# Blaizzy/mlx-audio

Hardware: NVIDIA H100
Metric: audio-sec/sec Kokoro-82M TTS (128-phoneme utterance, 9.75 s) (higher is better)
Workload: dtype bf16x2

## Files before the change

### mlx_audio_b200/csrc/lstm.cu

```cuda
#include "common.cuh"
#include <cooperative_groups.h>
#include <stdlib.h>
namespace cg = cooperative_groups;

namespace {

constexpr int LH = 256, NCTA = 8, UPC = LH / NCTA;

__global__ void __cluster_dims__(NCTA, 1, 1) __launch_bounds__(256, 1)
lstm_bidir_kernel(const float* __restrict__ xproj, const float* __restrict__ wh, float* __restrict__ out,
                  int64_t out_ld, int T) {
  cg::cluster_group cluster = cg::this_cluster();
  const int rank = (int)cluster.block_rank();
  const int dir = blockIdx.y, b = blockIdx.z;
  const int tid = threadIdx.x, half = tid & 1, r = tid >> 1;
  const int gate = r >> 5, unit = r & 31;
  const int grow = gate * LH + rank * UPC + unit;
  __shared__ __align__(16) float hbuf[2][LH];
  __shared__ float gates[4 * UPC];

  float w[128];
  {
    const float* wp = wh + ((int64_t)dir * 4 * LH + grow) * LH + half * 128;
#pragma unroll
    for (int j = 0; j < 128; j += 4) {
      float4 t = *reinterpret_cast<const float4*>(wp + j);
      w[j] = t.x; w[j + 1] = t.y; w[j + 2] = t.z; w[j + 3] = t.w;
    }
  }
  for (int i = tid; i < 2 * LH; i += 256) (&hbuf[0][0])[i] = 0.f;
  float c = 0.f;
  const float* xp_base = xproj + (int64_t)b * T * 2 * 4 * LH + (int64_t)dir * 4 * LH + grow;
  float xp_cur = 0.f;
  if (half == 0 && T > 0) xp_cur = __ldg(xp_base + (int64_t)(dir == 0 ? 0 : T - 1) * 2 * 4 * LH);
  cluster.sync();

  for (int step = 0; step < T; step++) {
    const int t = dir == 0 ? step : T - 1 - step;
    const int cur = step & 1;
    float xp_next = 0.f;
    if (half == 0 && step + 1 < T) xp_next = __ldg(xp_base + (int64_t)(dir == 0 ? t + 1 : t - 1) * 2 * 4 * LH);
    const float* hp = &hbuf[cur][half * 128];
    float s0 = 0.f, s1 = 0.f, s2 = 0.f, s3 = 0.f, s4 = 0.f, s5 = 0.f, s6 = 0.f, s7 = 0.f;
#pragma unroll
    for (int j = 0; j < 128; j += 8) {
      float4 a = *reinterpret_cast<const float4*>(hp + j);
      float4 e = *reinterpret_cast<const float4*>(hp + j + 4);
      s0 = fmaf(w[j], a.x, s0); s1 = fmaf(w[j + 1], a.y, s1); s2 = fmaf(w[j + 2], a.z, s2); s3 = fmaf(w[j + 3], a.w, s3);
      s4 = fmaf(w[j + 4], e.x, s4); s5 = fmaf(w[j + 5], e.y, s5); s6 = fmaf(w[j + 6], e.z, s6); s7 = fmaf(w[j + 7], e.w, s7);
    }
    float s = ((s0 + s1) + (s2 + s3)) + ((s4 + s5) + (s6 + s7));
    s += __shfl_xor_sync(0xffffffffu, s, 1);
    float* gbuf = gates + cur * (4 * UPC);
    if (half == 0) gbuf[r] = s + xp_cur;
    __syncthreads();
    if (tid < 4 * UPC) {
      const float v = gbuf[tid];
      gbuf[tid] = (tid >> 5) == 2 ? 1.f - __fdividef(2.f, 1.f + __expf(2.f * v)) : __fdividef(1.f, 1.f + __expf(-v));
      asm volatile("bar.sync 1, 128;" ::: "memory");
    }
    if (tid < UPC) {
      const float gi = gbuf[tid], gf = gbuf[UPC + tid], gg = gbuf[2 * UPC + tid], go = gbuf[3 * UPC + tid];
      c = fmaf(gf, c, gi * gg);
      const float hval = go * (1.f - __fdividef(2.f, 1.f + __expf(2.f * c)));
      out[((int64_t)b * T + t) * out_ld + dir * LH + rank * UPC + tid] = hval;
#pragma unroll
      for (int rr = 0; rr < NCTA; rr++) {
        float* remote = cluster.map_shared_rank(&hbuf[0][0], rr);
        remote[(cur ^ 1) * LH + rank * UPC + tid] = hval;
      }
    }
    xp_cur = xp_next;
    cluster.sync();
  }
}


__device__ __forceinline__ uint32_t smem_addr(const void* p) { return (uint32_t)__cvta_generic_to_shared(p); }
__device__ __forceinline__ uint32_t mapa(uint32_t addr, uint32_t rank) {
  uint32_t r; asm volatile("mapa.shared::cluster.u32 %0, %1, %2;" : "=r"(r) : "r"(addr), "r"(rank)); return r;
}
__device__ __forceinline__ void st_async_f32(uint32_t raddr, float v, uint32_t rbar) {
  asm volatile("st.async.weak.shared::cluster.mbarrier::complete_tx::bytes.b32 [%0], %1, [%2];"
               ::"r"(raddr), "r"(__float_as_uint(v)), "r"(rbar) : "memory");
}
__device__ __forceinline__ void bar_wait_cluster(uint32_t bar, uint32_t parity) {
  uint32_t ok = 0;
  while (!ok)
    asm volatile("{\n\t.reg .pred p;\n\tmbarrier.try_wait.parity.acquire.cluster.shared::cta.b64 p, [%1], %2;\n\tselp.u32 %0, 1, 0, p;\n\t}"
                 : "=r"(ok) : "r"(bar), "r"(parity) : "memory");
}

__global__ void __cluster_dims__(NCTA, 1, 1) __launch_bounds__(256, 1)
lstm_bidir_kernel_v2(const float* __restrict__ xproj, const float* __restrict__ wh, float* __restrict__ out,
                     int64_t out_ld, int T) {
  cg::cluster_group cluster = cg::this_cluster();
  const int rank = (int)cluster.block_rank();
  const int dir = blockIdx.y, b = blockIdx.z;
  const int tid = threadIdx.x, half = tid & 1, r = tid >> 1;
  const int gate = r >> 5, unit = r & 31;
  const int grow = gate * LH + rank * UPC + unit;
  __shared__ __align__(16) float hbuf[2][LH];
  __shared__ float gates[2 * 4 * UPC];
  __shared__ __align__(8) uint64_t hbar[2];

  float w[128];
  {
    const float* wp = wh + ((int64_t)dir * 4 * LH + grow) * LH + half * 128;
#pragma unroll
    for (int j = 0; j < 128; j += 4) {
      float4 t = *reinterpret_cast<const float4*>(wp + j);
      w[j] = t.x; w[j + 1] = t.y; w[j + 2] = t.z; w[j + 3] = t.w;
    }
  }
  for (int i = tid; i < 2 * LH; i += 256) (&hbuf[0][0])[i] = 0.f;
  if (tid == 0) {
    asm volatile("mbarrier.init.shared::cta.b64 [%0], 1;" ::"r"(smem_addr(&hbar[0])) : "memory");
    asm volatile("mbarrier.init.shared::cta.b64 [%0], 1;" ::"r"(smem_addr(&hbar[1])) : "memory");
    asm volatile("fence.mbarrier_init.release.cluster;" ::: "memory");
  }
  float c = 0.f;
  const float* xp_base = xproj + (int64_t)b * T * 2 * 4 * LH + (int64_t)dir * 4 * LH + grow;
  float xp_cur = 0.f;
  if (half == 0 && T > 0) xp_cur = __ldg(xp_base + (int64_t)(dir == 0 ? 0 : T - 1) * 2 * 4 * LH);
  uint32_t rh[NCTA], rb[NCTA];
  if (tid < UPC) {
#pragma unroll
    for (int q = 0; q < NCTA; q++) { rh[q] = mapa(smem_addr(&hbuf[0][0]), q); rb[q] = mapa(smem_addr(&hbar[0]), q); }
  }
  cluster.sync();

  for (int step = 0; step < T; step++) {
    const int t = dir == 0 ? step : T - 1 - step;
    const int cur = step & 1, nxt = cur ^ 1;
    if (tid == 0 && step + 1 < T)
      asm volatile("mbarrier.arrive.expect_tx.shared::cta.b64 _, [%0], %1;" ::"r"(smem_addr(&hbar[nxt])), "r"(NCTA * UPC * 4) : "memory");
    float xp_next = 0.f;
    if (half == 0 && step + 1 < T) xp_next = __ldg(xp_base + (int64_t)(dir == 0 ? t + 1 : t - 1) * 2 * 4 * LH);
    if (step > 0) bar_wait_cluster(smem_addr(&hbar[cur]), ((step - 1) >> 1) & 1);
    const float* hp = &hbuf[cur][half * 128];
    float s0 = 0.f, s1 = 0.f, s2 = 0.f, s3 = 0.f, s4 = 0.f, s5 = 0.f, s6 = 0.f, s7 = 0.f;
#pragma unroll
    for (int j = 0; j < 128; j += 8) {
      float4 a = *reinterpret_cast<const float4*>(hp + j);
      float4 e = *reinterpret_cast<const float4*>(hp + j + 4);
      s0 = fmaf(w[j], a.x, s0); s1 = fmaf(w[j + 1], a.y, s1); s2 = fmaf(w[j + 2], a.z, s2); s3 = fmaf(w[j + 3], a.w, s3);
      s4 = fmaf(w[j + 4], e.x, s4); s5 = fmaf(w[j + 5], e.y, s5); s6 = fmaf(w[j + 6], e.z, s6); s7 = fmaf(w[j + 7], e.w, s7);
    }
    float s = ((s0 + s1) + (s2 + s3)) + ((s4 + s5) + (s6 + s7));
    s += __shfl_xor_sync(0xffffffffu, s, 1);
    float* gbuf = gates + cur * (4 * UPC);
    if (half == 0) gbuf[r] = s + xp_cur;
    __syncthreads();
    if (tid < 4 * UPC) {
      const float v = gbuf[tid];
      gbuf[tid] = (tid >> 5) == 2 ? 1.f - __fdividef(2.f, 1.f + __expf(2.f * v)) : __fdividef(1.f, 1.f + __expf(-v));
      asm volatile("bar.sync 1, 128;" ::: "memory");
    }
    if (tid < UPC) {
      const float gi = gbuf[tid], gf = gbuf[UPC + tid], gg = gbuf[2 * UPC + tid], go = gbuf[3 * UPC + tid];
      c = fmaf(gf, c, gi * gg);
      const float hval = go * (1.f - __fdividef(2.f, 1.f + __expf(2.f * c)));
      out[((int64_t)b * T + t) * out_ld + dir * LH + rank * UPC + tid] = hval;
      const uint32_t off = (uint32_t)((nxt * LH + rank * UPC + tid) * 4);
      if (step + 1 < T) {
#pragma unroll
        for (int q = 0; q < NCTA; q++) st_async_f32(rh[q] + off, hval, rb[q] + (uint32_t)(nxt * 8));
      }
    }
    xp_cur = xp_next;
  }
  cluster.sync();
}

}

extern "C" int32_t b2a_lstm_bidir(const float* xproj, const float* wh, float* out, int64_t out_ld, int32_t B, int32_t T,
                                  int32_t H, void* stream) {
  B2A_CHECK_ARG(xproj && wh && out && B > 0 && T > 0, "bad pointers/shape");
  if (H != LH) { b2a_set_error("b2a_lstm_bidir: hidden size %d not supported (256)", H); return B2A_E_UNSUPPORTED; }
  dim3 grid(NCTA, 2, B);
  static int v2 = -1;
  if (v2 < 0) { const char* e = getenv("B2A_LSTM"); v2 = (e && e[0] == '1') ? 0 : 1; }
  if (v2) lstm_bidir_kernel_v2<<<grid, 256, 0, (cudaStream_t)stream>>>(xproj, wh, out, out_ld, T);
  else lstm_bidir_kernel<<<grid, 256, 0, (cudaStream_t)stream>>>(xproj, wh, out, out_ld, T);
  B2A_CHECK_LAUNCH();
  return B2A_OK;
}
```

Before: 1722.

## Restructure LSTM recurrence to warp-local gate reduction with vectorized cluster pushes

The LSTM step is remapped so that each warp owns four hidden units and all four of their gates. Each lane computes partial dot products over a 16-element slice of h, and a butterfly shuffle reduction produces the gate values. This removes the per-step __syncthreads, the named barrier and the shared gate buffer. The new hidden values are pushed to the other CTAs with one v4 st.async per destination, using a swizzled h layout, instead of 8 scalar stores per thread. The legacy kernel and its env-var fallback are removed, at the cost of more shuffles and more complex indexing.

```diff
diff --git a/mlx_audio_b200/csrc/lstm.cu b/mlx_audio_b200/csrc/lstm.cu
--- a/mlx_audio_b200/csrc/lstm.cu
+++ b/mlx_audio_b200/csrc/lstm.cu
@@ -1,88 +1,22 @@
 #include "common.cuh"
 #include <cooperative_groups.h>
-#include <stdlib.h>
 namespace cg = cooperative_groups;
 
 namespace {
 
 constexpr int LH = 256, NCTA = 8, UPC = LH / NCTA;
 
-__global__ void __cluster_dims__(NCTA, 1, 1) __launch_bounds__(256, 1)
-lstm_bidir_kernel(const float* __restrict__ xproj, const float* __restrict__ wh, float* __restrict__ out,
-                  int64_t out_ld, int T) {
-  cg::cluster_group cluster = cg::this_cluster();
-  const int rank = (int)cluster.block_rank();
-  const int dir = blockIdx.y, b = blockIdx.z;
-  const int tid = threadIdx.x, half = tid & 1, r = tid >> 1;
-  const int gate = r >> 5, unit = r & 31;
-  const int grow = gate * LH + rank * UPC + unit;
-  __shared__ __align__(16) float hbuf[2][LH];
-  __shared__ float gates[4 * UPC];
-
-  float w[128];
-  {
-    const float* wp = wh + ((int64_t)dir * 4 * LH + grow) * LH + half * 128;
-#pragma unroll
-    for (int j = 0; j < 128; j += 4) {
-      float4 t = *reinterpret_cast<const float4*>(wp + j);
-      w[j] = t.x; w[j + 1] = t.y; w[j + 2] = t.z; w[j + 3] = t.w;
-    }
-  }
-  for (int i = tid; i < 2 * LH; i += 256) (&hbuf[0][0])[i] = 0.f;
-  float c = 0.f;
-  const float* xp_base = xproj + (int64_t)b * T * 2 * 4 * LH + (int64_t)dir * 4 * LH + grow;
-  float xp_cur = 0.f;
-  if (half == 0 && T > 0) xp_cur = __ldg(xp_base + (int64_t)(dir == 0 ? 0 : T - 1) * 2 * 4 * LH);
-  cluster.sync();
-
-  for (int step = 0; step < T; step++) {
-    const int t = dir == 0 ? step : T - 1 - step;
-    const int cur = step & 1;
-    float xp_next = 0.f;
-    if (half == 0 && step + 1 < T) xp_next = __ldg(xp_base + (int64_t)(dir == 0 ? t + 1 : t - 1) * 2 * 4 * LH);
-    const float* hp = &hbuf[cur][half * 128];
-    float s0 = 0.f, s1 = 0.f, s2 = 0.f, s3 = 0.f, s4 = 0.f, s5 = 0.f, s6 = 0.f, s7 = 0.f;
-#pragma unroll
-    for (int j = 0; j < 128; j += 8) {
-      float4 a = *reinterpret_cast<const float4*>(hp + j);
-      float4 e = *reinterpret_cast<const float4*>(hp + j + 4);
-      s0 = fmaf(w[j], a.x, s0); s1 = fmaf(w[j + 1], a.y, s1); s2 = fmaf(w[j + 2], a.z, s2); s3 = fmaf(w[j + 3], a.w, s3);
-      s4 = fmaf(w[j + 4], e.x, s4); s5 = fmaf(w[j + 5], e.y, s5); s6 = fmaf(w[j + 6], e.z, s6); s7 = fmaf(w[j + 7], e.w, s7);
-    }
-    float s = ((s0 + s1) + (s2 + s3)) + ((s4 + s5) + (s6 + s7));
-    s += __shfl_xor_sync(0xffffffffu, s, 1);
-    float* gbuf = gates + cur * (4 * UPC);
-    if (half == 0) gbuf[r] = s + xp_cur;
-    __syncthreads();
-    if (tid < 4 * UPC) {
-      const float v = gbuf[tid];
-      gbuf[tid] = (tid >> 5) == 2 ? 1.f - __fdividef(2.f, 1.f + __expf(2.f * v)) : __fdividef(1.f, 1.f + __expf(-v));
-      asm volatile("bar.sync 1, 128;" ::: "memory");
-    }
-    if (tid < UPC) {
-      const float gi = gbuf[tid], gf = gbuf[UPC + tid], gg = gbuf[2 * UPC + tid], go = gbuf[3 * UPC + tid];
-      c = fmaf(gf, c, gi * gg);
-      const float hval = go * (1.f - __fdividef(2.f, 1.f + __expf(2.f * c)));
-      out[((int64_t)b * T + t) * out_ld + dir * LH + rank * UPC + tid] = hval;
-#pragma unroll
-      for (int rr = 0; rr < NCTA; rr++) {
-        float* remote = cluster.map_shared_rank(&hbuf[0][0], rr);
-        remote[(cur ^ 1) * LH + rank * UPC + tid] = hval;
-      }
-    }
-    xp_cur = xp_next;
-    cluster.sync();
-  }
-}
-
+__device__ __forceinline__ int hslot(int p) { return p ^ (((p >> 5) & 3) << 2); }
+__device__ __forceinline__ int slot_column(int p) { return ((p >> 7) << 7) | ((p & 15) << 3) | ((p >> 4) & 7); }
 
 __device__ __forceinline__ uint32_t smem_addr(const void* p) { return (uint32_t)__cvta_generic_to_shared(p); }
 __device__ __forceinline__ uint32_t mapa(uint32_t addr, uint32_t rank) {
   uint32_t r; asm volatile("mapa.shared::cluster.u32 %0, %1, %2;" : "=r"(r) : "r"(addr), "r"(rank)); return r;
 }
-__device__ __forceinline__ void st_async_f32(uint32_t raddr, float v, uint32_t rbar) {
-  asm volatile("st.async.weak.shared::cluster.mbarrier::complete_tx::bytes.b32 [%0], %1, [%2];"
-               ::"r"(raddr), "r"(__float_as_uint(v)), "r"(rbar) : "memory");
+__device__ __forceinline__ void st_async_v4(uint32_t raddr, float4 v, uint32_t rbar) {
+  asm volatile("st.async.weak.shared::cluster.mbarrier::complete_tx::bytes.v4.b32 [%0], {%1, %2, %3, %4}, [%5];"
+               ::"r"(raddr), "r"(__float_as_uint(v.x)), "r"(__float_as_uint(v.y)), "r"(__float_as_uint(v.z)), "r"(__float_as_uint(v.w)),
+                 "r"(rbar) : "memory");
 }
 __device__ __forceinline__ void bar_wait_cluster(uint32_t bar, uint32_t parity) {
   uint32_t ok = 0;
@@ -92,25 +26,28 @@
 }
 
 __global__ void __cluster_dims__(NCTA, 1, 1) __launch_bounds__(256, 1)
-lstm_bidir_kernel_v2(const float* __restrict__ xproj, const float* __restrict__ wh, float* __restrict__ out,
-                     int64_t out_ld, int T) {
+lstm_bidir_kernel(const float* __restrict__ xproj, const float* __restrict__ wh, float* __restrict__ out, int64_t out_ld, int T) {
   cg::cluster_group cluster = cg::this_cluster();
   const int rank = (int)cluster.block_rank();
   const int dir = blockIdx.y, b = blockIdx.z;
-  const int tid = threadIdx.x, half = tid & 1, r = tid >> 1;
-  const int gate = r >> 5, unit = r & 31;
-  const int grow = gate * LH + rank * UPC + unit;
+  const int tid = threadIdx.x, lane = tid & 31, warp = tid >> 5;
+  const int k = lane & 7, half = (lane >> 3) & 1, grp = lane >> 4;
+  const int p0 = rank * UPC + warp * 4;
+  const int hk = half * 8 + k;
+  const int gate = ((lane >> 1) & 1) * 2 + ((lane >> 2) & 1);
+  const int unit = slot_column(p0 + grp * 2 + (lane & 1));
   __shared__ __align__(16) float hbuf[2][LH];
-  __shared__ float gates[2 * 4 * UPC];
   __shared__ __align__(8) uint64_t hbar[2];
 
-  float w[128];
-  {
-    const float* wp = wh + ((int64_t)dir * 4 * LH + grow) * LH + half * 128;
+  float w[8][16];
 #pragma unroll
-    for (int j = 0; j < 128; j += 4) {
-      float4 t = *reinterpret_cast<const float4*>(wp + j);
-      w[j] = t.x; w[j + 1] = t.y; w[j + 2] = t.z; w[j + 3] = t.w;
+  for (int u = 0; u < 2; u++) {
+    const int ju = slot_column(p0 + grp * 2 + u);
+#pragma unroll
+    for (int g = 0; g < 4; g++) {
+      const float* wp = wh + ((int64_t)dir * 4 * LH + g * LH + ju) * LH + half * 128 + k;
+#pragma unroll
+      for (int i = 0; i < 16; i++) w[u * 4 + g][i] = __ldg(wp + 8 * i);
     }
   }
   for (int i = tid; i < 2 * LH; i += 256) (&hbuf[0][0])[i] = 0.f;
@@ -120,14 +57,11 @@
     asm volatile("fence.mbarrier_init.release.cluster;" ::: "memory");
   }
   float c = 0.f;
-  const float* xp_base = xproj + (int64_t)b * T * 2 * 4 * LH + (int64_t)dir * 4 * LH + grow;
-  float xp_cur = 0.f;
-  if (half == 0 && T > 0) xp_cur = __ldg(xp_base + (int64_t)(dir == 0 ? 0 : T - 1) * 2 * 4 * LH);
-  uint32_t rh[NCTA], rb[NCTA];
-  if (tid < UPC) {
-#pragma unroll
-    for (int q = 0; q < NCTA; q++) { rh[q] = mapa(smem_addr(&hbuf[0][0]), q); rb[q] = mapa(smem_addr(&hbar[0]), q); }
-  }
+  const float* xp_base = xproj + (int64_t)b * T * 2 * 4 * LH + (int64_t)dir * 4 * LH + gate * LH + unit;
+  float xp_cur = __ldg(xp_base + (int64_t)(dir == 0 ? 0 : T - 1) * 2 * 4 * LH);
+  uint32_t rh = 0, rb = 0;
+  if (lane < NCTA) { rh = mapa(smem_addr(&hbuf[0][0]), lane); rb = mapa(smem_addr(&hbar[0]), lane); }
+  const uint32_t push_off = (uint32_t)hslot(p0) * 4;
   cluster.sync();
 
   for (int step = 0; step < T; step++) {
@@ -136,38 +70,42 @@
     if (tid == 0 && step + 1 < T)
       asm volatile("mbarrier.arrive.expect_tx.shared::cta.b64 _, [%0], %1;" ::"r"(smem_addr(&hbar[nxt])), "r"(NCTA * UPC * 4) : "memory");
     float xp_next = 0.f;
-    if (half == 0 && step + 1 < T) xp_next = __ldg(xp_base + (int64_t)(dir == 0 ? t + 1 : t - 1) * 2 * 4 * LH);
+    if (step + 1 < T) xp_next = __ldg(xp_base + (int64_t)(dir == 0 ? t + 1 : t - 1) * 2 * 4 * LH);
     if (step > 0) bar_wait_cluster(smem_addr(&hbar[cur]), ((step - 1) >> 1) & 1);
-    const float* hp = &hbuf[cur][half * 128];
-    float s0 = 0.f, s1 = 0.f, s2 = 0.f, s3 = 0.f, s4 = 0.f, s5 = 0.f, s6 = 0.f, s7 = 0.f;
+    float hv[16];
 #pragma unroll
-    for (int j = 0; j < 128; j += 8) {
-      float4 a = *reinterpret_cast<const float4*>(hp + j);
-      float4 e = *reinterpret_cast<const float4*>(hp + j + 4);
-      s0 = fmaf(w[j], a.x, s0); s1 = fmaf(w[j + 1], a.y, s1); s2 = fmaf(w[j + 2], a.z, s2); s3 = fmaf(w[j + 3], a.w, s3);
-      s4 = fmaf(w[j + 4], e.x, s4); s5 = fmaf(w[j + 5], e.y, s5); s6 = fmaf(w[j + 6], e.z, s6); s7 = fmaf(w[j + 7], e.w, s7);
+    for (int m = 0; m < 4; m++) {
+      const float4 a = *reinterpret_cast<const float4*>(&hbuf[cur][hslot(hk * 16 + 4 * m)]);
+      hv[4 * m] = a.x; hv[4 * m + 1] = a.y; hv[4 * m + 2] = a.z; hv[4 * m + 3] = a.w;
     }
-    float s = ((s0 + s1) + (s2 + s3)) + ((s4 + s5) + (s6 + s7));
-    s += __shfl_xor_sync(0xffffffffu, s, 1);
-    float* gbuf = gates + cur * (4 * UPC);
-    if (half == 0) gbuf[r] = s + xp_cur;
-    __syncthreads();
-    if (tid < 4 * UPC) {
-      const float v = gbuf[tid];
-      gbuf[tid] = (tid >> 5) == 2 ? 1.f - __fdividef(2.f, 1.f + __expf(2.f * v)) : __fdividef(1.f, 1.f + __expf(-v));
-      asm volatile("bar.sync 1, 128;" ::: "memory");
+    float s[8];
+#pragma unroll
+    for (int r = 0; r < 8; r++) s[r] = 0.f;
+#pragma unroll
+    for (int i = 0; i < 16; i++) {
+#pragma unroll
+      for (int r = 0; r < 8; r++) s[r] = fmaf(w[r][i], hv[i], s[r]);
     }
-    if (tid < UPC) {
-      const float gi = gbuf[tid], gf = gbuf[UPC + tid], gg = gbuf[2 * UPC + tid], go = gbuf[3 * UPC + tid];
-      c = fmaf(gf, c, gi * gg);
-      const float hval = go * (1.f - __fdividef(2.f, 1.f + __expf(2.f * c)));
-      out[((int64_t)b * T + t) * out_ld + dir * LH + rank * UPC + tid] = hval;
-      const uint32_t off = (uint32_t)((nxt * LH + rank * UPC + tid) * 4);
-      if (step + 1 < T) {
+    const bool b0 = lane & 1, b1 = lane & 2, b2 = lane & 4;
+    float s4[4], s2[2];
 #pragma unroll
-        for (int q = 0; q < NCTA; q++) st_async_f32(rh[q] + off, hval, rb[q] + (uint32_t)(nxt * 8));
-      }
-    }
+    for (int j = 0; j < 4; j++) s4[j] = (b0 ? s[4 + j] : s[j]) + __shfl_xor_sync(0xffffffffu, b0 ? s[j] : s[4 + j], 1);
+#pragma unroll
+    for (int j = 0; j < 2; j++) s2[j] = (b1 ? s4[2 + j] : s4[j]) + __shfl_xor_sync(0xffffffffu, b1 ? s4[j] : s4[2 + j], 2);
+    float sh = (b2 ? s2[1] : s2[0]) + __shfl_xor_sync(0xffffffffu, b2 ? s2[0] : s2[1], 4);
+    float v = sh + __shfl_xor_sync(0xffffffffu, sh, 8);
+    v = v + xp_cur;
+    const float a = gate == 2 ? 1.f - __fdividef(2.f, 1.f + __expf(2.f * v)) : __fdividef(1.f, 1.f + __expf(-v));
+    const int src = (lane & 0x19);
+    const float gi = __shfl_sync(0xffffffffu, a, src), gf = __shfl_sync(0xffffffffu, a, src + 4);
+    const float gg = __shfl_sync(0xffffffffu, a, src + 2), go = __shfl_sync(0xffffffffu, a, src + 6);
+    c = fmaf(gf, c, gi * gg);
+    const float hval = go * (1.f - __fdividef(2.f, 1.f + __expf(2.f * c)));
+    if ((lane & 0xe) == 0) out[((int64_t)b * T + t) * out_ld + dir * LH + unit] = hval;
+    const float4 h4 = make_float4(__shfl_sync(0xffffffffu, hval, 0), __shfl_sync(0xffffffffu, hval, 1),
+                                  __shfl_sync(0xffffffffu, hval, 16), __shfl_sync(0xffffffffu, hval, 17));
+    if (lane < NCTA && step + 1 < T)
+      st_async_v4(rh + (uint32_t)(nxt * LH * 4) + push_off, h4, rb + (uint32_t)(nxt * 8));
     xp_cur = xp_next;
   }
   cluster.sync();
@@ -179,11 +117,7 @@
                                   int32_t H, void* stream) {
   B2A_CHECK_ARG(xproj && wh && out && B > 0 && T > 0, "bad pointers/shape");
   if (H != LH) { b2a_set_error("b2a_lstm_bidir: hidden size %d not supported (256)", H); return B2A_E_UNSUPPORTED; }
-  dim3 grid(NCTA, 2, B);
-  static int v2 = -1;
-  if (v2 < 0) { const char* e = getenv("B2A_LSTM"); v2 = (e && e[0] == '1') ? 0 : 1; }
-  if (v2) lstm_bidir_kernel_v2<<<grid, 256, 0, (cudaStream_t)stream>>>(xproj, wh, out, out_ld, T);
-  else lstm_bidir_kernel<<<grid, 256, 0, (cudaStream_t)stream>>>(xproj, wh, out, out_ld, T);
+  lstm_bidir_kernel<<<dim3(NCTA, 2, B), 256, 0, (cudaStream_t)stream>>>(xproj, wh, out, out_ld, T);
   B2A_CHECK_LAUNCH();
   return B2A_OK;
 }
```

New measurement: 1777 (median of 6 runs). +3.2%, better.
